# Shigangli/Ok-Topk

Measured on NVIDIA H100. Metric: train_samples_per_sec_vgg16_oktopk_density0.001, higher is better.
Workload: dtype fp32

## Files before the change

### oktopk_b200/config.py

```python
from __future__ import annotations

import dataclasses
from dataclasses import dataclass, field
from typing import Dict, Optional, Sequence


@dataclass
class OkTopkConfig:
    compressor: str = "oktopk"
    density: float = 0.01
    sparse: bool = True

    bucket_elems: int = 64 * 1024 * 1024

    warmup_iters: int = 0
    local_recompute_interval: int = 32
    global_recompute_interval: int = 32
    repartition_interval: int = 64
    topkaopt_recompute_interval: int = 32

    overselect_guard_num: int = 4
    overselect_guard_den: int = 3
    overselect_guard_factor: float = 1.03
    overselect_guard_loops: int = 5
# ... 8 lines not shown
    global_adapt_inc: float = 1.008
    global_adapt_dec: float = 1.008

    throttle: int = 4
    balanced_allgather: bool = False
    dsa_dense_fallback_frac: float = 1.0 / 3.0

    gaussian_low: float = 3.0 / 4.0
    gaussian_high: float = 5.0 / 4.0
    gaussian_factor: float = 1.02
    gaussian_loops: int = 20
    gaussian_mode: str = "vgg"

    sigma_scale: float = 2.5
    norm_clip: Optional[float] = None
    dynamic_densities: Optional[Sequence[float]] = None

    backend: str = "auto"
    fused: bool = True
    deterministic: bool = False
    slot_factor: float = 0.0
    gather_factor: float = 0.0
    dense_switch_density: float = 0.05
    max_redo: int = 12
    redo_factor: float = 1.5
    land_grads: bool = True
    nvls: str = "auto"
    comm_ctas: int = 0
    pull_mode: str = "tma"
    overlap: bool = True
    early_pack: bool = True
    early_pack_frac: float = 0.85
    early_pack_ctas: int = 32
    gselect_mode: str = "auto"
    peer_timeout_s: float = 60.0

    def k_for(self, numel: int, density: Optional[float] = None) -> int:
        d = self.density if density is None else density
        return int(numel * d)

    def replace(self, **kw) -> "OkTopkConfig":
        return dataclasses.replace(self, **kw)

    def to_dict(self) -> Dict:
        return dataclasses.asdict(self)


@dataclass(frozen=True)
class LossScale:
    init_scale: float = 2.0 ** 16
    growth_factor: float = 2.0
    backoff_factor: float = 0.5
    growth_interval: int = 2000

    def __post_init__(self):
        if not (self.init_scale > 0 and self.growth_factor >= 1 and 0 < self.backoff_factor <= 1
                and self.growth_interval >= 1):
            raise ValueError("LossScale: need init_scale > 0, growth_factor >= 1, 0 < backoff_factor <= 1, "
                             "growth_interval >= 1")

    @staticmethod
    def parse(spec) -> Optional["LossScale"]:
        if spec is None or isinstance(spec, LossScale):
            return spec
        if isinstance(spec, str) and spec.strip().lower() == "dynamic":
            return LossScale()
# ... 62 lines not shown
```

### oktopk_b200/csrc/bindings.cpp

```cpp
#include <pybind11/pybind11.h>
#include <pybind11/stl.h>
#include <cuda.h>
#include <cuda_runtime.h>

#include <unistd.h>

#include <algorithm>
#include <cstring>
#include <stdexcept>
#include <string>
#include <tuple>
#include <vector>

#include "oktopk.cuh"

namespace py = pybind11;
using namespace okt;

static void ck(cudaError_t e, const char* what) {
    if (e != cudaSuccess) throw std::runtime_error(std::string(what) + ": " + cudaGetErrorString(e));
}
template <class T> static T* P_(uint64_t p) { return reinterpret_cast<T*>(p); }
static cudaStream_t S_(uint64_t s) { return reinterpret_cast<cudaStream_t>(s); }

// ... 419 lines not shown
    }
}

static void dense_run(const std::vector<uint64_t>& bufs, const std::vector<uint64_t>& flags, uint64_t epoch, int n,
                      int rank, int grid, uint64_t stream, uint64_t st, double timeout_s, uint64_t mc,
                      uint64_t host_fault, uint64_t skip) {
    DenseParams p;
    std::memset(&p, 0, sizeof(p));
    if (bufs.size() > OKT_MAXP || bufs.size() != flags.size()) throw std::runtime_error("bad peer tables");
    for (size_t i = 0; i < bufs.size(); ++i) { p.bufs[i] = P_<float>(bufs[i]); p.flags[i] = P_<uint64_t>(flags[i]); }
    p.epoch = P_<unsigned long long>(epoch);
    p.n = n; p.P = (int)bufs.size(); p.rank = rank; p.scale = 1.0f / (float)p.P;
    p.fault = st ? &P_<OktState>(st)->fault : nullptr;
    p.timeout_ns = (unsigned long long)(timeout_s * 1e9);
    p.mc = P_<float>(mc);
    p.host_fault = P_<int>(host_fault);
    p.skip = P_<const int>(skip);
    ck(launch_dense_allreduce(p, grid, S_(stream)), "dense allreduce launch");
}

static void kth_abs(uint64_t x, int n, int k, uint64_t st, uint64_t out, int grid, uint64_t stream) {
    ck(launch_kth_abs(P_<float>(x), n, k, P_<OktState>(st), P_<float>(out), grid, S_(stream)), "kth_abs launch");
}

static void fused_sgd(uint64_t p, uint64_t g, uint64_t mom, int n, double momentum, double dampening, double wd,
                      int nesterov, int first, int zero_grad, uint64_t stream, uint64_t scal_ptr, uint64_t fault_ptr,
                      uint64_t skip_ptr) {
    if (scal_ptr == 0) throw std::runtime_error("fused_sgd: scal_ptr must point at the group's device scalars");
    ck(launch_fused_sgd(P_<float>(p), P_<float>(g), P_<float>(mom), n, (float)momentum, (float)dampening, (float)wd,
                        nesterov, first, zero_grad, P_<float>(scal_ptr), P_<int>(fault_ptr), P_<int>(skip_ptr),
                        S_(stream)),
       "fused_sgd");
}
static void fused_bert_adam(uint64_t p, uint64_t g, uint64_t m, uint64_t v, int n, double b1, double b2, double eps,
                            double wd, int zero_grad, uint64_t stream, uint64_t scal_ptr, uint64_t fault_ptr,
                            uint64_t skip_ptr) {
    if (scal_ptr == 0) throw std::runtime_error("fused_bert_adam: scal_ptr must point at the group's device scalars");
    ck(launch_fused_bert_adam(P_<float>(p), P_<float>(g), P_<float>(m), P_<float>(v), n, (float)b1, (float)b2,
                              (float)eps, (float)wd, zero_grad, P_<float>(scal_ptr), P_<int>(fault_ptr), P_<int>(skip_ptr),
                              S_(stream)),
       "fused_bert_adam");
}
static void fused_adam(uint64_t p, uint64_t g, uint64_t m, uint64_t v, int n, double beta1, double beta2, double eps,
                       double wd, int decoupled, int zero_grad, uint64_t stream, uint64_t scal_ptr, uint64_t fault_ptr,
                       uint64_t skip_ptr) {
    if (scal_ptr == 0) throw std::runtime_error("fused_adam: scal_ptr must point at the group's device scalars");
    ck(launch_fused_adam(P_<float>(p), P_<float>(g), P_<float>(m), P_<float>(v), n, beta1, beta2, (float)eps, (float)wd,
                         decoupled, zero_grad, P_<float>(scal_ptr), P_<int>(fault_ptr), P_<int>(skip_ptr), S_(stream)),
       "fused_adam");
}
static Dtype dtype_arg(int dtype, const char* what) {
    if (dtype < 0 || dtype > 2) throw std::runtime_error(std::string(what) + ": dtype must be 0 (fp32), 1 (bf16) or 2 (fp16)");
    return static_cast<Dtype>(dtype);
}
static void bn_forward(uint64_t x, uint64_t y, uint64_t arg, uint64_t partial, uint64_t gamma, uint64_t beta, uint64_t cbias,
                       uint64_t save_mean, uint64_t save_invstd, uint64_t rmean, uint64_t rvar, uint64_t nbt, double momentum,
                       double eps, int relu, int M, int C, int W, int slot, int max_ctas, uint64_t stream, int dtype,
                       uint64_t res) {
    if (C % 4 != 0) throw std::runtime_error("bn_forward: channel count must be a multiple of 4");
    if (slot < 0) throw std::runtime_error("bn_forward: negative slot");
    if (res != 0 && (W != 0 || !relu)) throw std::runtime_error("bn_forward: a residual needs relu = 1 and no pool");
    ck(launch_bn_forward(P_<const void>(x), P_<void>(y), P_<unsigned char>(arg), P_<float>(partial), P_<const float>(gamma),
                         P_<const float>(beta), P_<const float>(cbias), P_<float>(save_mean), P_<float>(save_invstd),
                         P_<float>(rmean), P_<float>(rvar), P_<long long>(nbt), (float)momentum, (float)eps, relu, M, C, W, slot,
                         max_ctas, dtype_arg(dtype, "bn_forward"), S_(stream), P_<const void>(res)), "bn_forward");
}
// ... 221 lines not shown
    m.def("max_coop_grid", &okt_max_coop_grid);
    m.def("oktopk_run", &oktopk_run);
    m.def("gather_run", &gather_run);
    m.def("dense_run", &dense_run, py::arg("bufs"), py::arg("flags"), py::arg("epoch"), py::arg("n"), py::arg("rank"),
          py::arg("grid"), py::arg("stream"), py::arg("st") = 0, py::arg("timeout_s") = 0.0, py::arg("mc") = 0,
          py::arg("host_fault") = 0, py::arg("skip") = 0);
    m.def("gtopk_run", &gtopk_run);
    m.def("land_grads", &land_grads);
    m.def("read_trace", &read_trace);
    m.def("host_flag_alloc", &host_flag_alloc);
    m.def("host_flag_free", &host_flag_free);
    m.def("host_flag_read", &host_flag_read);
    m.def("host_flag_clear", &host_flag_clear);
    m.def("fault_ptr", [](uint64_t st) { return (uint64_t)&P_<OktState>(st)->fault; });
    m.def("gather_max_coop_grid", &gather_max_coop_grid);
    m.def("gtopk_max_coop_grid", &gtopk_max_coop_grid);
    m.def("vmm_probe", &vmm_probe);
    m.def("vmm_create", &vmm_create);
    m.def("vmm_import", &vmm_import);
    m.def("vmm_map", &vmm_map);
    m.def("vmm_unmap", &vmm_unmap);
    m.def("vmm_release", &vmm_release);
    m.def("mc_create", &mc_create);
    m.def("mc_add_device", &mc_add_device);
    m.def("mc_bind", &mc_bind);
    m.def("close_fd", [](int fd) { if (fd >= 0) ::close(fd); });
    m.def("clear_fault", [](uint64_t st, uint64_t stream) {
        ck(cudaMemsetAsync(&P_<OktState>(st)->fault, 0, sizeof(int), S_(stream)), "clear_fault");
    });
    m.def("kth_abs", &kth_abs);
    m.def("fused_sgd", &fused_sgd, py::arg("p"), py::arg("g"), py::arg("mom"), py::arg("n"), py::arg("momentum"),
          py::arg("dampening"), py::arg("wd"), py::arg("nesterov"), py::arg("first"), py::arg("zero_grad"),
          py::arg("stream"), py::arg("scal_ptr"), py::arg("fault_ptr") = 0, py::arg("skip_ptr") = 0);
    m.def("fused_bert_adam", &fused_bert_adam, py::arg("p"), py::arg("g"), py::arg("m"), py::arg("v"), py::arg("n"),
          py::arg("b1"), py::arg("b2"), py::arg("eps"), py::arg("wd"), py::arg("zero_grad"), py::arg("stream"),
          py::arg("scal_ptr"), py::arg("fault_ptr") = 0, py::arg("skip_ptr") = 0);
    m.def("fused_adam", &fused_adam, py::arg("p"), py::arg("g"), py::arg("m"), py::arg("v"), py::arg("n"),
          py::arg("beta1"), py::arg("beta2"), py::arg("eps"), py::arg("wd"), py::arg("decoupled"), py::arg("zero_grad"),
          py::arg("stream"), py::arg("scal_ptr"), py::arg("fault_ptr") = 0, py::arg("skip_ptr") = 0);
    m.def("momentum_correct", &momentum_correct);
    m.def("unscale_check", &unscale_check);
    m.def("scale_update", [](uint64_t ls, double growth, double backoff, int interval, uint64_t stream) {
        ck(launch_scale_update(P_<LossScaleDev>(ls), growth, backoff, interval, S_(stream)), "scale_update");
    });
    m.def("adam_scalars", [](uint64_t ls, uint64_t hyper, uint64_t scal, int groups, uint64_t stream) {
        ck(launch_adam_scalars(P_<const LossScaleDev>(ls), P_<const double>(hyper), P_<float>(scal), groups, S_(stream)),
           "adam_scalars");
    });
    m.def("carry_residual", [](uint64_t g, uint64_t res, int n, uint64_t skip, uint64_t stream) {
        ck(launch_carry_residual(P_<float>(g), P_<float>(res), n, P_<const int>(skip), S_(stream)), "carry_residual");
    });
    m.attr("LOSS_SCALE_BYTES") = sizeof(LossScaleDev);
    m.attr("SCALE_SYNC_BYTES") = sizeof(ScaleSync);
    m.attr("VERDICT_OFFSET") = offsetof(ScaleSync, verdict);
    m.def("maxpool2_fwd", &maxpool2_fwd);
    m.def("maxpool2_bwd", &maxpool2_bwd);
    m.def("bn_forward", &bn_forward, py::arg("x"), py::arg("y"), py::arg("arg"), py::arg("partial"), py::arg("gamma"),
          py::arg("beta"), py::arg("cbias"), py::arg("save_mean"), py::arg("save_invstd"), py::arg("rmean"), py::arg("rvar"),
          py::arg("nbt"), py::arg("momentum"), py::arg("eps"), py::arg("relu"), py::arg("M"), py::arg("C"), py::arg("W"),
          py::arg("slot"), py::arg("max_ctas"), py::arg("stream"), py::arg("dtype"), py::arg("res") = 0);
    m.def("bn_backward", &bn_backward, py::arg("x"), py::arg("dy"), py::arg("arg"), py::arg("dx"), py::arg("partial"),
          py::arg("gamma"), py::arg("beta"), py::arg("save_mean"), py::arg("save_invstd"), py::arg("dgamma"), py::arg("dbeta"),
          py::arg("relu"), py::arg("M"), py::arg("C"), py::arg("W"), py::arg("slot"), py::arg("max_ctas"), py::arg("stream"),
          py::arg("dtype"), py::arg("res") = 0, py::arg("dres") = 0);
    m.def("bn_tile_rows", &bn_tile_rows);
    m.def("bn_sliced", &bn_sliced, py::arg("M"), py::arg("C"), py::arg("W"));
// ... 47 lines not shown
```

### oktopk_b200/csrc/oktopk.cuh

```cuda
#pragma once
#include <cuda_runtime.h>
#include <stdint.h>
#include <stddef.h>

#ifndef OKT_MAXP
#define OKT_MAXP 16
#endif

namespace okt {

constexpr int kThreads = 512;
constexpr int kWarps = kThreads / 32;
constexpr int kChunk = 1024;
constexpr int kHistBins = 2048;
constexpr int kMaxWarpsTotal = 16384;
constexpr int kGuardMax = 64;
constexpr int kGuardFineMax = 15;
constexpr int kCtasPerSm = 1;
constexpr int kPackTile = 2;
constexpr int kPackStages = 4;
constexpr int kPackSmemBytes = kPackStages * 2 * kPackTile * kThreads * 16;
constexpr int kScanStages = 2 * kPackStages;
constexpr int kStrideGridMax = 132 * 8;

// ... 194 lines not shown
    int ccap;
    int* sel_idx;
    float* sel_val;
    int selcap;
    int* host_fault;
    const int* skip;
};

struct DenseParams {
    float* bufs[OKT_MAXP];
    uint64_t* flags[OKT_MAXP];
    unsigned long long* epoch;
    int n, P, rank;
    float scale;
    int* fault;
    unsigned long long timeout_ns;
    float* mc;
    int* host_fault;
    const int* skip;
};

int okt_max_coop_grid(int device);
cudaError_t launch_oktopk(const OktParams& p, int grid, cudaStream_t stream);
cudaError_t launch_oktopk_segment(const OktParams& p, int max_ctas, cudaStream_t stream);
cudaError_t launch_gather_scheme(const GatherParams& p, int grid, cudaStream_t stream);
cudaError_t launch_gtopk(const TreeParams& p, int grid, cudaStream_t stream);
int gtopk_max_coop_grid(int device);
int gather_max_coop_grid(int device);
cudaError_t launch_dense_allreduce(const DenseParams& p, int grid, cudaStream_t stream);
cudaError_t launch_kth_abs(const float* x, int n, int k, OktState* st, float* out_thr, int grid, cudaStream_t stream);
cudaError_t launch_fused_sgd(float* p, float* g, float* mom, int n, float momentum, float dampening, float weight_decay,
                             int nesterov, int first_step, int zero_grad, const float* scal, const int* fault,
                             const int* skip, cudaStream_t stream);
cudaError_t launch_fused_bert_adam(float* p, float* g, float* m, float* v, int n, float b1, float b2, float eps,
                                   float weight_decay, int zero_grad, const float* scal, const int* fault,
                                   const int* skip, cudaStream_t stream);
cudaError_t launch_fused_adam(float* p, float* g, float* m, float* v, int n, double beta1, double beta2, float eps,
                              float weight_decay, int decoupled, int zero_grad, const float* scal, const int* fault,
                              const int* skip, cudaStream_t stream);

struct LossScaleDev {
    float scale;
    float inv_scale;
    int growth_tracker;
    int found_inf;
    long long skipped;
    long long adam_step;
};
struct ScaleSync {
    int flag;
    unsigned int ticket;
    unsigned int epoch;
    int verdict;
};
constexpr int kScaleThreads = 256;
constexpr int kScalePerCta = 8192;
struct ScaleParams {
    LossScaleDev* ls;
    ScaleSync* sync;
    int* fault;
    int* host_fault;
    char* peers[OKT_MAXP];
    size_t mbox_off;
    int P, rank;
    unsigned long long timeout_ns;
    int nseg;
// ... 76 lines not shown
```

### oktopk_b200/csrc/optim.cu

```cuda
#include "common.cuh"
#include "oktopk.cuh"

namespace okt {

constexpr int kOptThreads = 256;

template <int kScal, int kState, typename Upd>
__device__ __forceinline__ void update_pass(float* __restrict__ p, float* __restrict__ g, float* __restrict__ m,
                                            float* __restrict__ v, int n, bool load, bool store, int zero_grad,
                                            const float* __restrict__ scal, const int* __restrict__ fault,
                                            const int* __restrict__ skip, Upd upd) {
    if (fault != nullptr && *reinterpret_cast<const volatile int*>(fault) != 0) return;
    const int n4 = n >> 2;
    float4* p4 = reinterpret_cast<float4*>(p);
    float4* g4 = reinterpret_cast<float4*>(g);
    float4* m4 = reinterpret_cast<float4*>(m);
    float4* v4 = reinterpret_cast<float4*>(v);
    const float4 zero = make_float4(0.f, 0.f, 0.f, 0.f);
    if (verdict_set(skip)) {
        if (!zero_grad) return;
        for (int i = blockIdx.x * kOptThreads + threadIdx.x; i < n4; i += gridDim.x * kOptThreads) {
            const float4 gw = ld_stream_f4(g4 + i);
            if (gw.x != 0.f || gw.y != 0.f || gw.z != 0.f || gw.w != 0.f) g4[i] = zero;
        }
// ... 6 lines not shown
    for (int j = 0; j < kScal; ++j) s[j] = scal[j];
    for (int i = blockIdx.x * kOptThreads + threadIdx.x; i < n4; i += gridDim.x * kOptThreads) {
        float4 pw = p4[i], gw = ld_stream_f4(g4 + i), mw = zero, vw = zero;
        if (load) {
            mw = m4[i];
            if (kState == 2) vw = v4[i];
        }
        upd(s, pw.x, gw.x, mw.x, vw.x); upd(s, pw.y, gw.y, mw.y, vw.y);
        upd(s, pw.z, gw.z, mw.z, vw.z); upd(s, pw.w, gw.w, mw.w, vw.w);
        p4[i] = pw;
        if (store) {
            m4[i] = mw;
            if (kState == 2) v4[i] = vw;
        }
        if (zero_grad && (gw.x != 0.f || gw.y != 0.f || gw.z != 0.f || gw.w != 0.f)) g4[i] = zero;
    }
    if (blockIdx.x == 0)
        for (int i = n4 * 4 + threadIdx.x; i < n; i += kOptThreads) {
            float pw = p[i], gw = g[i], mw = 0.f, vw = 0.f;
            if (load) {
                mw = m[i];
                if (kState == 2) vw = v[i];
            }
            upd(s, pw, gw, mw, vw);
            p[i] = pw;
            if (store) {
                m[i] = mw;
                if (kState == 2) v[i] = vw;
            }
            if (zero_grad) g[i] = 0.f;
        }
}

__global__ void __launch_bounds__(kOptThreads) fused_sgd_kernel(float* __restrict__ p, float* __restrict__ g,
                                                                 float* __restrict__ mom, int n, float momentum,
                                                                 float dampening, float wd, int nesterov, int first,
                                                                 int zero_grad, const float* __restrict__ scal,
                                                                 const int* __restrict__ fault,
                                                                 const int* __restrict__ skip) {
    const float damp = first ? 0.f : dampening;
    update_pass<1, 1>(p, g, mom, nullptr, n, momentum != 0.f && !first, momentum != 0.f, zero_grad, scal, fault, skip,
                      [=](const float* s, float& pw, float gw, float& mw, float&) {
                          float d = __fmaf_rn(wd, pw, gw);
                          if (momentum != 0.f) {
                              mw = first ? d : __fmaf_rn(1.f - damp, d, __fmul_rn(momentum, mw));
                              d = nesterov ? __fmaf_rn(momentum, mw, d) : mw;
                          }
                          pw = __fmaf_rn(-s[0], d, pw);
                      });
}

__global__ void __launch_bounds__(kOptThreads) fused_bert_adam_kernel(float* __restrict__ p, float* __restrict__ g,
                                                                       float* __restrict__ m, float* __restrict__ v,
                                                                       int n, float b1, float b2, float eps, float wd,
                                                                       int zero_grad, const float* __restrict__ scal,
                                                                       const int* __restrict__ fault,
                                                                       const int* __restrict__ skip) {
    update_pass<1, 2>(p, g, m, v, n, true, true, zero_grad, scal, fault, skip,
                      [=](const float* s, float& pw, float gw, float& mw, float& vw) {
                          mw = b1 * mw + (1.f - b1) * gw;
                          vw = b2 * vw + (1.f - b2) * gw * gw;
                          float u = mw / (sqrtf(vw) + eps);
                          if (wd > 0.f) u += wd * pw;
                          pw -= s[0] * u;
                      });
}

__global__ void __launch_bounds__(kOptThreads) fused_adam_kernel(float* __restrict__ p, float* __restrict__ g,
                                                                  float* __restrict__ m, float* __restrict__ v, int n,
                                                                  float w, float b2, float omb2, float eps, float wd,
                                                                  int decoupled, int zero_grad,
                                                                  const float* __restrict__ scal,
                                                                  const int* __restrict__ fault,
                                                                  const int* __restrict__ skip) {
    const bool small_w = fabsf(w) < 0.5f;
    const float lw = small_w ? w : 1.f - w;
    update_pass<3, 2>(p, g, m, v, n, true, true, zero_grad, scal, fault, skip,
                      [=](const float* s, float& pw, float gw, float& mw, float& vw) {
                          const float decay = s[0], step_size = s[1], bc2_sqrt = s[2];
                          if (decoupled) pw = pw * decay;
                          else if (wd != 0.f) gw = gw + wd * pw;
                          mw = small_w ? mw + lw * (gw - mw) : gw - (gw - mw) * lw;
// ... 18 lines not shown
    for (int i = blockIdx.x * kOptThreads + threadIdx.x; i < n; i += gridDim.x * kOptThreads) {
        double v = (double)x[i];
        acc += v * v;
    }
    acc = warp_sum_d(acc);
    __shared__ double s[kOptThreads / 32];
    if ((threadIdx.x & 31) == 0) s[threadIdx.x >> 5] = acc;
    __syncthreads();
    if (threadIdx.x < 32) {
        double v = (threadIdx.x < kOptThreads / 32) ? s[threadIdx.x] : 0.0;
        v = warp_sum_d(v);
        if (threadIdx.x == 0) atomicAdd(out, (float)v);
    }
}

__global__ void __launch_bounds__(kOptThreads) clip_scale_kernel(float* __restrict__ x, int n, const float* norm_sq,
                                                                  float max_norm) {
    const float nrm = sqrtf(*norm_sq);
    if (!(nrm > max_norm) || nrm == 0.f) return;
    const float s = max_norm / nrm;
    for (int i = blockIdx.x * kOptThreads + threadIdx.x; i < n; i += gridDim.x * kOptThreads) x[i] *= s;
}

static inline int opt_grid(int n) {
    int g = (n / 4 + kOptThreads - 1) / kOptThreads;
    if (g < 1) g = 1;
    if (g > kStrideGridMax) g = kStrideGridMax;
    return g;
}

cudaError_t launch_fused_sgd(float* p, float* g, float* mom, int n, float momentum, float dampening, float weight_decay,
                             int nesterov, int first_step, int zero_grad, const float* scal, const int* fault,
                             const int* skip, cudaStream_t stream) {
    fused_sgd_kernel<<<opt_grid(n), kOptThreads, 0, stream>>>(p, g, mom, n, momentum, dampening, weight_decay, nesterov,
                                                             first_step, zero_grad, scal, fault, skip);
    return cudaGetLastError();
}

cudaError_t launch_fused_bert_adam(float* p, float* g, float* m, float* v, int n, float b1, float b2, float eps,
                                   float weight_decay, int zero_grad, const float* scal, const int* fault,
                                   const int* skip, cudaStream_t stream) {
    fused_bert_adam_kernel<<<opt_grid(n), kOptThreads, 0, stream>>>(p, g, m, v, n, b1, b2, eps, weight_decay, zero_grad,
                                                                   scal, fault, skip);
    return cudaGetLastError();
}

cudaError_t launch_fused_adam(float* p, float* g, float* m, float* v, int n, double beta1, double beta2, float eps,
                              float weight_decay, int decoupled, int zero_grad, const float* scal, const int* fault,
                              const int* skip, cudaStream_t stream) {
    fused_adam_kernel<<<opt_grid(n), kOptThreads, 0, stream>>>(p, g, m, v, n, (float)(1.0 - beta1), (float)beta2,
                                                              (float)(1.0 - beta2), eps, weight_decay, decoupled,
                                                              zero_grad, scal, fault, skip);
    return cudaGetLastError();
}

constexpr int kLandThreads = 256;
constexpr int kLandPerCta = 8192;

__global__ void __launch_bounds__(kLandThreads) land_kernel(const LandParams lp, float* __restrict__ bucket) {
    int lo = 0, hi = lp.count - 1;
    while (lo < hi) {
        const int mid = (lo + hi + 1) >> 1;
        if ((int)blockIdx.x >= lp.blk_begin[mid]) lo = mid; else hi = mid - 1;
    }
    const int t = lo;
    const int part = blockIdx.x - lp.blk_begin[t];
    const float* __restrict__ src = lp.src[t];
    float* __restrict__ dst = bucket + lp.dst_off[t];
// ... 43 lines not shown
```

### oktopk_b200/ops/ext.py

```python
from __future__ import annotations

import importlib
import os
from typing import Optional

import torch

_C = None
_ERR: Optional[BaseException] = None

LAUNCH_COUNT = {"total": 0}
_LAUNCHERS = {"oktopk_run": 1, "gather_run": 1, "gtopk_run": 1, "dense_run": 1, "kth_abs": 1, "fused_sgd": 1,
              "fused_bert_adam": 1, "fused_adam": 1, "momentum_correct": 1, "clip_by_norm": 2, "land_grads": 1, "bn_forward": 1, "bn_backward": 1,
              "maxpool2_fwd": 1, "maxpool2_bwd": 1, "unscale_check": 1, "ln_forward": 1, "ln_backward": 2,
              "xent_forward": 2, "xent_backward": 1, "lstm_forward": 1, "lstm_backward": 1, "mlm_select": 1,
              "mlm_gather": 1, "mlm_scatter": 1, "attn_forward": 1, "attn_backward": 2, "lstm_seq_forward": 1,
              "lstm_seq_backward": 1}


class _CountingModule:

    def __init__(self, mod):
        self._mod = mod
        for name, per_call in _LAUNCHERS.items():
            setattr(self, name, self._wrap(getattr(mod, name), name, per_call))

    def _wrap(self, fn, name, per_call):
        def call(*a, **kw):
            n = per_call
            if name == "oktopk_run" and isinstance(a[9], dict) and a[9].get("split_phases"):
                n = 7
            if name == "land_grads":
                n = max(1, (len(a[0]) + 95) // 96)
            LAUNCH_COUNT["total"] += n
            LAUNCH_COUNT[name] = LAUNCH_COUNT.get(name, 0) + n
            return fn(*a, **kw)
        return call

    def __getattr__(self, name):
        return getattr(self._mod, name)


def load(build_if_missing: bool = True):
    global _C, _ERR
    if _C is not None:
        return _C
# ... 47 lines not shown
```

### oktopk_b200/optimizer.py

```python
from __future__ import annotations

import math
import warnings
from typing import Dict, Iterable, List, Optional

import torch

from .compression import NoneCompressor, compressors, resolve_compressor
from .config import LossScale, OkTopkConfig
from .ops import ext
from .parallel.allreducer import AllReducer
from .parallel.buckets import Bucket, attach, build_buckets
from .parallel.early_pack import PackPlanner
from .parallel.world import World, world as _world


class _ScaleState:

    def __init__(self, ls: LossScale, device: torch.device):
        self.cfg = ls
        self.buf = torch.zeros(32, dtype=torch.uint8, device=device)
        self.f32 = self.buf[0:8].view(torch.float32)
        self.i32 = self.buf[8:16].view(torch.int32)
        self.i64 = self.buf[16:32].view(torch.int64)
        self.native = device.type == "cuda" and ext.available()
        self.reset()

    @property
    def ptr(self) -> int:
        return self.buf.data_ptr()

    @property
    def found_ptr(self) -> int:
        return self.buf.data_ptr() + 12

    def reset(self, scale: Optional[float] = None, growth_tracker: int = 0, skipped: int = 0, adam_step: int = 0) -> None:
        from .parallel.oracle import inv_scale_of
        scale = self.cfg.init_scale if scale is None else scale
        vals = torch.zeros(32, dtype=torch.uint8)
        vals[0:8].view(torch.float32).copy_(torch.tensor([scale, inv_scale_of(scale)], dtype=torch.float32))
        vals[8:16].view(torch.int32).copy_(torch.tensor([growth_tracker, 0], dtype=torch.int32))
        vals[16:32].view(torch.int64).copy_(torch.tensor([skipped, adam_step], dtype=torch.int64))
        self.buf.copy_(vals)

    def scale(self) -> torch.Tensor:
        return self.f32[0]

# ... 63 lines not shown
        self._use_streams = False
        self._land = False
        for b in self._buckets:
            dev = b.params[0].device
            grad = allreducer.register_bucket(b.name, b.numel, dev)
            attach(b, grad, flatten_params)
            if dev.type == "cuda" and self._cfg.land_grads and ext.available():
                self._land = True
            b.pending = len(b.params)
            b.dirty = False
            if dev.type == "cuda":
                self._use_streams = self._cfg.overlap
                b.event = torch.cuda.Event()
            for p in b.params:
                self._bucket_of[p] = b
                self._hook_handles.append(p.register_post_accumulate_grad_hook(self._make_hook(p)))
        if self._update is _AdamUpdate:
            if not (ext.available() and all(b.flat_param is not None and b.grad.is_cuda for b in self._buckets)):
                self._update = None
        self._direct = (self._land and self._update is not None and allreducer.compressor.name == "oktopk"
                        and all(b.flat_param is not None for b in self._buckets))
        self._packs = {}
        self._pos_in_bucket = {p: i for b in self._buckets for i, p in enumerate(b.params)}
        if self._direct and self._use_streams:
            for b in self._buckets:
                if len(b.params) <= ext.require().SRC_SEG_MAX:
                    self._packs[b.index] = PackPlanner(b.offsets, b.numel,
                                                       math.ceil(self._cfg.early_pack_frac * b.numel),
                                                       ext.require().PACK_RANGE_MAX)
            for b in self._buckets:
                b.packing = None
        if self._use_streams:
            self._comm_stream = torch.cuda.Stream(priority=-1)
        allreducer.add_resync_hook(self._resync_replicas)
        if loss_scale is not None:
            allreducer.enable_loss_scaling()
            self._ls = _ScaleState(loss_scale, self._buckets[0].params[0].device if self._buckets else torch.device("cpu"))
        self._lr_dev = self._hyper_dev = None
        self._lr_pin, self._lr_ev, self._lr_ring, self._lr_last = [], [], 0, None
        dev0 = self._buckets[0].params[0].device if self._buckets else torch.device("cpu")
        if dev0.type == "cuda" and ext.available() and self._update is not None:
            groups = max(len(self.param_groups), 1)
            self._lr_dev = torch.zeros(groups * self._update.n_scalars, dtype=torch.float32, device=dev0)
            stage = self._lr_dev
            if self._ls is not None and self._update is _AdamUpdate:
                stage = self._hyper_dev = torch.zeros(groups * 4, dtype=torch.float64, device=dev0)
            self._lr_pin = [torch.zeros_like(stage, device="cpu").pin_memory() for _ in range(8)]
            self._lr_ev = [None] * len(self._lr_pin)

    def _resync_replicas(self) -> None:
        w = self._allreducer.world
        if w.size == 1:
            return
        for b in self._buckets:
            if b.flat_param is not None:
                w.broadcast(b.flat_param, 0)
            else:
                for p in b.params:
                    w.broadcast(p.data, 0)
            for t in self._flat_state.get(b.index, {}).values():
                if torch.is_tensor(t):
                    w.broadcast(t, 0)

    @property
    def _okt_adam(self) -> bool:
        return self._update is _AdamUpdate
# ... 30 lines not shown
            b = self._bucket_of[p]
            b.dirty = True
            if self.local:
                return
            b.pending -= 1
            if b.pending == 0:
                self._launch_ready()
            elif b.index in self._packs:
                self._pack_early(b, p)
        return hook

    def _pack_early(self, b: Bucket, p) -> None:
        if b.packing is None:
            b.packing = (self._direct and not self.momentum_correction and self._ls is None
                         and self._allreducer.reads_sources(b.name) and self._allreducer.packs_early(b.name))
        if not b.packing:
            return
        planner = self._packs[b.index]
        ranges = planner.ready(self._pos_in_bucket[p])
        if ranges is None:
            return
        ptrs, offs, lens = [], [], []
        for q, o, v in sorted(zip(b.params, b.offsets, b.grad_views), key=lambda t: t[1]):
            g = q.grad
            if not any(lo <= o < hi for lo, hi in ranges) or g is None or g.numel() == 0:
                continue
            if (g.data_ptr() == v.data_ptr() or g.dtype != torch.float32 or not g.is_cuda or g.stride() != v.stride()
                    or g.data_ptr() % 16):
                raise RuntimeError("early pack: the gradient of %s cannot be read in place; set "
                                   "OkTopkConfig.early_pack=False" % self._parameter_names.get(q, "?"))
            ptrs.append(g.data_ptr())
            offs.append(o)
            lens.append(g.numel())
        ev = torch.cuda.Event()
        ev.record(torch.cuda.current_stream())
        self._comm_stream.wait_event(ev)
        with torch.cuda.stream(self._comm_stream):
            self._allreducer.pack_segment(b.name, ranges, (ptrs, offs, lens), stream=self._comm_stream)

    def _launch_ready(self) -> None:
        while self._next_launch < len(self._buckets) and self._buckets[self._next_launch].pending <= 0:
            self._launch(self._buckets[self._next_launch])
            self._next_launch += 1

    def _land_bucket(self, b: Bucket) -> None:
        srcs, offs, numels = [], [], []
        for p, o, v in zip(b.params, b.offsets, b.grad_views):
            g = p.grad
            if g is None:
                srcs.append(0)
                offs.append(o)
                numels.append(p.numel())
            elif g.data_ptr() == v.data_ptr():
                continue
            elif g.dtype == torch.float32 and g.is_cuda and g.stride() == v.stride():
                srcs.append(g.data_ptr())
                offs.append(o)
                numels.append(g.numel())
            else:
                v.copy_(g)
            p.grad = v
        if srcs:
            ext.require().land_grads(srcs, offs, numels, b.grad.data_ptr(), torch.cuda.current_stream().cuda_stream)

    def _source_table(self, b: Bucket):
        ptrs, offs, lens, held = [], [], [], []
        for p, o, v in zip(b.params, b.offsets, b.grad_views):
            g = p.grad
            if g is None or g.numel() == 0:
                continue
            if (g.data_ptr() == v.data_ptr() or g.dtype != torch.float32 or not g.is_cuda or g.stride() != v.stride()
# ... 67 lines not shown
        return loss * self._ls.scale()

    def loss_scale_state(self) -> Optional[Dict]:
        if self._ls is None:
            return None
        st = self._ls.state()
        return {k: st[k] for k in ("scale", "growth_tracker", "skipped_steps")}

    def _scale_state_dict(self) -> Optional[Dict]:
        if self._ls is None:
            return None
        st = self._ls.state()
        st.pop("found_inf")
        return st

    def _load_scale_state(self, sd: Optional[Dict], adam_step: int) -> None:
        if self._ls is None:
            return
        if sd is None:
            self._ls.reset(adam_step=adam_step)
        else:
            self._ls.reset(sd["scale"], sd["growth_tracker"], sd["skipped_steps"], sd.get("adam_step", adam_step))

    def synchronize(self) -> None:
        if self._synced:
            return
        for b in self._buckets:
            b.pending = 0
        self._launch_ready()
        if self._comm_stream is not None:
            cur = torch.cuda.current_stream()
            for b in self._buckets:
                cur.wait_event(b.event)
        for b in self._buckets:
            b.held = None
        self._synced = True

    def _after_step(self) -> None:
        for b in self._buckets:
            b.pending = len(b.params)
            b.launched = False
            if b.index in self._packs:
                self._packs[b.index].reset()
                b.packing = None
        self._next_launch = 0
        self._synced = False
        self._allreducer.poll_faults()

    def _clear_buckets(self) -> None:
        if self._direct:
            with torch.no_grad():
                for b in self._buckets:
                    b.grad.zero_()

    def zero_grad(self, set_to_none: bool = False) -> None:
        if self._land:
            for b in self._buckets:
                for p in b.params:
                    p.grad = None
                b.dirty = False
            return
        for b in self._buckets:
            if b.dirty:
                b.grad.zero_()
                b.dirty = False

    def stop(self) -> None:
        self._allreducer.stop()

    def add_train_epoch(self) -> None:
        self._allreducer.train_epoch += 1

    def get_current_density(self) -> float:
        return self._allreducer.get_current_density()

    def comm_stats(self) -> Dict:
        return self._allreducer.stats()
# ... 23 lines not shown
        else:
            self._maybe_refresh_lr()
            if self._hyper_dev is not None and self._update is _AdamUpdate:
                ext.require().adam_scalars(self._ls.ptr, self._hyper_dev.data_ptr(), self._lr_dev.data_ptr(),
                                           len(self.param_groups), torch.cuda.current_stream().cuda_stream)
            with torch.no_grad():
                for b in self._buckets:
                    self._fused_update(b, host_skip)
            self.counter += 1
        if self._ls is not None:
            self._ls.update()
        self._after_step()
        return loss

    def _device_update(self) -> bool:
        return self._update is not None and self._lr_dev is not None and all(
            b.grad.is_cuda and b.flat_param is not None for b in self._buckets)

    def _flat_buffers(self, b: Bucket) -> Dict[str, torch.Tensor]:
        fs = self._flat_state.setdefault(b.index, {})
        for k in self._update.keys:
            if k not in fs:
                fs[k] = torch.zeros_like(b.grad)
                for p, v in zip(b.params, b.views(fs[k])):
                    self.state[p][k] = v
        return fs

    def _fused_update(self, b: Bucket, host_skip: bool = False) -> None:
        first = self._update.keys[0] not in self._flat_state.get(b.index, {})
        fs = self._flat_buffers(b)
        on_gpu = b.grad.is_cuda and b.flat_param is not None and ext.available()
        zero_grad = 0 if self._land and not self._direct else 1
        skip_ptr = self._ls.found_ptr if self._ls is not None else 0
        for gi, s, e in b.group_slices:
            def launch(fn, *hyper):
                fn(b.flat_param.data_ptr() + 4 * s, b.grad.data_ptr() + 4 * s,
                   *(fs[k].data_ptr() + 4 * s for k in self._update.keys), e - s, *hyper, zero_grad,
                   torch.cuda.current_stream().cuda_stream, self._lr_ptr(gi), self._allreducer.fault_ptr(b.name),
                   skip_ptr)
            if on_gpu or not host_skip:
                self._update.update(self, b, self.param_groups[gi], s, e, fs, first, launch if on_gpu else None)
            if not on_gpu:
                b.grad[s:e].zero_()
        b.dirty = False

    def _adopt_state(self, counter: Optional[int] = None) -> None:
        keys = self._update.keys
        have = {p for b in self._buckets for p in b.params if self.state.get(p, {}).get(keys[0]) is not None}
        if counter is None:
            steps = {float(self.state[p]["step"]) for p in have if "step" in self.state[p]}
            if len(steps) > 1:
                warnings.warn("DistributedOptimizer: the loaded Adam state has unequal step counts per parameter %s; "
                              "using torch's Adam step from now on" % sorted(steps))
                self._update = None
                self._clear_buckets()
                self._direct = False
                for b in self._buckets:
                    for k in keys:
                        self._flat_state.get(b.index, {}).pop(k, None)
                return
            counter = int(steps.pop()) if steps else 0
        self.counter = counter
        loaded = {(p, k): self.state[p][k] for p in have for k in keys}
        with torch.no_grad():
            for b in self._buckets:
                for p in b.params:
                    self.state.get(p, {}).pop("step", None)
                if not any(p in have for p in b.params):
                    for k in keys:
                        self._flat_state.get(b.index, {}).pop(k, None)
                    continue
                fs = self._flat_buffers(b)
                for k in keys:
                    for p, v in zip(b.params, b.views(fs[k])):
                        if p in have:
                            v.copy_(loaded[p, k])
                        else:
                            v.zero_()
                        self.state[p][k] = v


class _SGDUpdate:
    keys = ("momentum_buffer",)
    n_scalars = 1

    @staticmethod
    def scalars(opt, g):
        return (float(g["lr"]),)

    @staticmethod
    def update(opt, b, g, s, e, fs, first, launch):
        lr, m, damp, wd, nest = g["lr"], g.get("momentum", 0.0), g.get("dampening", 0.0), \
            g.get("weight_decay", 0.0), bool(g.get("nesterov", False))
        if opt.momentum_correction:
            m = 0.0
        if launch is not None:
            launch(ext.require().fused_sgd, m, damp, wd, int(nest), int(first))
            return
        gs, ms = b.grad[s:e], fs["momentum_buffer"][s:e]
        if b.flat_param is not None:
            _SGDUpdate.math(b.flat_param[s:e], gs, ms, lr, m, damp, wd, nest, first)
        else:
            for p, o in zip(b.params, b.offsets):
                if s <= o < e:
                    _SGDUpdate.math(p.data.view(-1), gs[o - s:o - s + p.numel()], ms[o - s:o - s + p.numel()],
                                    lr, m, damp, wd, nest, first)

    @staticmethod
    def math(p, g, mom, lr, m, damp, wd, nest, first) -> None:
        d = g.add(p, alpha=wd) if wd != 0 else g.clone()
        if m != 0:
            if first:
                mom.copy_(d)
            else:
                mom.mul_(m).add_(d, alpha=1 - damp)
            d = d.add(mom, alpha=m) if nest else mom
        p.add_(d, alpha=-lr)


class _AdamUpdate:
    keys = ("exp_avg", "exp_avg_sq")
    n_scalars = 3

    @staticmethod
    def scalars(opt, g):
        if opt._hyper_dev is not None:
            return (float(g["lr"]), float(g["weight_decay"]), float(g["betas"][0]), float(g["betas"][1]))
        lr, (b1, b2), t = float(g["lr"]), g["betas"], float(opt.counter + 1)
# ... 235 lines not shown
```

Baseline: 14410.

## Precompute zero-gradient SGD step for early-packed ranges on a side stream

For ranges packed early during backward, a side-stream kernel stashes the params and momentum, then applies the SGD step as if the gradient were zero. It runs limited to a few CTAs so it overlaps with backward and communication. After the allreduce, a tail kernel redoes the update from the stash only where the gradient vector is nonzero, and runs the full update on the remaining dense ranges. This aims to take most of the optimizer's memory traffic off the critical path with very sparse gradients. The cost is two extra stash buffers, added side-stream contention with compute, and extra fault/skip handling that restores the stashed values.

```diff
diff --git a/oktopk_b200/config.py b/oktopk_b200/config.py
--- a/oktopk_b200/config.py
+++ b/oktopk_b200/config.py
@@ -64,6 +64,7 @@
     early_pack: bool = True
     early_pack_frac: float = 0.85
     early_pack_ctas: int = 32
+    sgd_ahead: bool = True
     gselect_mode: str = "auto"
     peer_timeout_s: float = 60.0
 
diff --git a/oktopk_b200/csrc/bindings.cpp b/oktopk_b200/csrc/bindings.cpp
--- a/oktopk_b200/csrc/bindings.cpp
+++ b/oktopk_b200/csrc/bindings.cpp
@@ -475,6 +475,45 @@
                         S_(stream)),
        "fused_sgd");
 }
+static SgdRanges sgd_ranges(const std::vector<std::pair<long long, long long>>& rs, int n, const char* what) {
+    if ((int)rs.size() > kPackRangeMax)
+        throw std::runtime_error(std::string(what) + ": more than " + std::to_string(kPackRangeMax) + " ranges");
+    SgdRanges r;
+    std::memset(&r, 0, sizeof(r));
+    r.nr = (int)rs.size();
+    for (int q = 0; q < r.nr; ++q) {
+        const long long lo = rs[q].first, hi = rs[q].second;
+        if (lo < 0 || hi < lo || lo % 4 || hi % 4 || hi > 4LL * (n / 4))
+            throw std::runtime_error(std::string(what) + ": ranges must lie at multiples of 4 inside the slice's whole "
+                                     "float4 vectors");
+        r.lo[q] = (int)(lo / 4);
+        r.hi[q] = (int)(hi / 4);
+    }
+    return r;
+}
+static void sgd_ahead(uint64_t p, uint64_t mom, uint64_t sp, uint64_t sm, int n,
+                      const std::vector<std::pair<long long, long long>>& ranges, double momentum, double dampening,
+                      double wd, int nesterov, int max_ctas, uint64_t stream, uint64_t scal_ptr) {
+    if (scal_ptr == 0) throw std::runtime_error("sgd_ahead: scal_ptr must point at the group's device scalars");
+    if (momentum != 0.0 && (mom == 0 || sm == 0)) throw std::runtime_error("sgd_ahead: momentum needs mom and sm");
+    const SgdHyper h{(float)momentum, (float)dampening, (float)wd, nesterov, 0};
+    ck(launch_sgd_ahead(P_<float>(p), P_<float>(mom), P_<float>(sp), P_<float>(sm), sgd_ranges(ranges, n, "sgd_ahead"),
+                        h, max_ctas, P_<float>(scal_ptr), S_(stream)),
+       "sgd_ahead");
+}
+static void fused_sgd_tail(uint64_t p, uint64_t g, uint64_t mom, uint64_t sp, uint64_t sm, int n,
+                           const std::vector<std::pair<long long, long long>>& ahead,
+                           const std::vector<std::pair<long long, long long>>& dense, double momentum, double dampening,
+                           double wd, int nesterov, int first, int zero_grad, uint64_t stream, uint64_t scal_ptr,
+                           uint64_t fault_ptr, uint64_t skip_ptr) {
+    if (scal_ptr == 0) throw std::runtime_error("fused_sgd_tail: scal_ptr must point at the group's device scalars");
+    if (momentum != 0.0 && (mom == 0 || sm == 0)) throw std::runtime_error("fused_sgd_tail: momentum needs mom and sm");
+    const SgdHyper h{(float)momentum, (float)dampening, (float)wd, nesterov, first};
+    ck(launch_fused_sgd_tail(P_<float>(p), P_<float>(g), P_<float>(mom), P_<const float>(sp), P_<const float>(sm), n,
+                             sgd_ranges(ahead, n, "fused_sgd_tail"), sgd_ranges(dense, n, "fused_sgd_tail"), h,
+                             zero_grad, P_<float>(scal_ptr), P_<int>(fault_ptr), P_<int>(skip_ptr), S_(stream)),
+       "fused_sgd_tail");
+}
 static void fused_bert_adam(uint64_t p, uint64_t g, uint64_t m, uint64_t v, int n, double b1, double b2, double eps,
                             double wd, int zero_grad, uint64_t stream, uint64_t scal_ptr, uint64_t fault_ptr,
                             uint64_t skip_ptr) {
@@ -762,6 +801,13 @@
     m.def("fused_sgd", &fused_sgd, py::arg("p"), py::arg("g"), py::arg("mom"), py::arg("n"), py::arg("momentum"),
           py::arg("dampening"), py::arg("wd"), py::arg("nesterov"), py::arg("first"), py::arg("zero_grad"),
           py::arg("stream"), py::arg("scal_ptr"), py::arg("fault_ptr") = 0, py::arg("skip_ptr") = 0);
+    m.def("sgd_ahead", &sgd_ahead, py::arg("p"), py::arg("mom"), py::arg("sp"), py::arg("sm"), py::arg("n"),
+          py::arg("ranges"), py::arg("momentum"), py::arg("dampening"), py::arg("wd"), py::arg("nesterov"),
+          py::arg("max_ctas"), py::arg("stream"), py::arg("scal_ptr"));
+    m.def("fused_sgd_tail", &fused_sgd_tail, py::arg("p"), py::arg("g"), py::arg("mom"), py::arg("sp"), py::arg("sm"),
+          py::arg("n"), py::arg("ahead"), py::arg("dense"), py::arg("momentum"), py::arg("dampening"), py::arg("wd"),
+          py::arg("nesterov"), py::arg("first"), py::arg("zero_grad"), py::arg("stream"), py::arg("scal_ptr"),
+          py::arg("fault_ptr") = 0, py::arg("skip_ptr") = 0);
     m.def("fused_bert_adam", &fused_bert_adam, py::arg("p"), py::arg("g"), py::arg("m"), py::arg("v"), py::arg("n"),
           py::arg("b1"), py::arg("b2"), py::arg("eps"), py::arg("wd"), py::arg("zero_grad"), py::arg("stream"),
           py::arg("scal_ptr"), py::arg("fault_ptr") = 0, py::arg("skip_ptr") = 0);
diff --git a/oktopk_b200/csrc/oktopk.cuh b/oktopk_b200/csrc/oktopk.cuh
--- a/oktopk_b200/csrc/oktopk.cuh
+++ b/oktopk_b200/csrc/oktopk.cuh
@@ -250,6 +250,20 @@
 cudaError_t launch_fused_sgd(float* p, float* g, float* mom, int n, float momentum, float dampening, float weight_decay,
                              int nesterov, int first_step, int zero_grad, const float* scal, const int* fault,
                              const int* skip, cudaStream_t stream);
+struct SgdRanges {
+    int nr;
+    int lo[kPackRangeMax];
+    int hi[kPackRangeMax];
+};
+struct SgdHyper {
+    float momentum, dampening, wd;
+    int nesterov, first;
+};
+cudaError_t launch_sgd_ahead(float* p, float* mom, float* sp, float* sm, const SgdRanges& r, const SgdHyper& h,
+                             int max_ctas, const float* scal, cudaStream_t stream);
+cudaError_t launch_fused_sgd_tail(float* p, float* g, float* mom, const float* sp, const float* sm, int n,
+                                  const SgdRanges& ahead, const SgdRanges& dense, const SgdHyper& h, int zero_grad,
+                                  const float* scal, const int* fault, const int* skip, cudaStream_t stream);
 cudaError_t launch_fused_bert_adam(float* p, float* g, float* m, float* v, int n, float b1, float b2, float eps,
                                    float weight_decay, int zero_grad, const float* scal, const int* fault,
                                    const int* skip, cudaStream_t stream);
diff --git a/oktopk_b200/csrc/optim.cu b/oktopk_b200/csrc/optim.cu
--- a/oktopk_b200/csrc/optim.cu
+++ b/oktopk_b200/csrc/optim.cu
@@ -62,22 +62,138 @@
         }
 }
 
+__device__ __forceinline__ void sgd_update(const SgdHyper& h, float lr, float& pw, float gw, float& mw) {
+    const float damp = h.first ? 0.f : h.dampening;
+    float d = __fmaf_rn(h.wd, pw, gw);
+    if (h.momentum != 0.f) {
+        mw = h.first ? d : __fmaf_rn(1.f - damp, d, __fmul_rn(h.momentum, mw));
+        d = h.nesterov ? __fmaf_rn(h.momentum, mw, d) : mw;
+    }
+    pw = __fmaf_rn(-lr, d, pw);
+}
+
+__device__ __forceinline__ void sgd_update4(const SgdHyper& h, float lr, float4& pw, const float4& gw, float4& mw) {
+    sgd_update(h, lr, pw.x, gw.x, mw.x); sgd_update(h, lr, pw.y, gw.y, mw.y);
+    sgd_update(h, lr, pw.z, gw.z, mw.z); sgd_update(h, lr, pw.w, gw.w, mw.w);
+}
+
 __global__ void __launch_bounds__(kOptThreads) fused_sgd_kernel(float* __restrict__ p, float* __restrict__ g,
-                                                                 float* __restrict__ mom, int n, float momentum,
-                                                                 float dampening, float wd, int nesterov, int first,
+                                                                 float* __restrict__ mom, int n, const SgdHyper h,
                                                                  int zero_grad, const float* __restrict__ scal,
                                                                  const int* __restrict__ fault,
                                                                  const int* __restrict__ skip) {
-    const float damp = first ? 0.f : dampening;
-    update_pass<1, 1>(p, g, mom, nullptr, n, momentum != 0.f && !first, momentum != 0.f, zero_grad, scal, fault, skip,
-                      [=](const float* s, float& pw, float gw, float& mw, float&) {
-                          float d = __fmaf_rn(wd, pw, gw);
-                          if (momentum != 0.f) {
-                              mw = first ? d : __fmaf_rn(1.f - damp, d, __fmul_rn(momentum, mw));
-                              d = nesterov ? __fmaf_rn(momentum, mw, d) : mw;
-                          }
-                          pw = __fmaf_rn(-s[0], d, pw);
-                      });
+    update_pass<1, 1>(p, g, mom, nullptr, n, h.momentum != 0.f && !h.first, h.momentum != 0.f, zero_grad, scal, fault,
+                      skip, [=](const float* s, float& pw, float gw, float& mw, float&) { sgd_update(h, s[0], pw, gw, mw); });
+}
+
+constexpr int kAheadUnroll = 4;
+
+__device__ __forceinline__ void st_evict_f4(float4* p, const float4& v) {
+    asm volatile("st.global.cs.v4.f32 [%0], {%1,%2,%3,%4};" ::"l"(p), "f"(v.x), "f"(v.y), "f"(v.z), "f"(v.w) : "memory");
+}
+
+__global__ void __launch_bounds__(kOptThreads) sgd_ahead_kernel(float* __restrict__ p, float* __restrict__ mom,
+                                                                 float* __restrict__ sp, float* __restrict__ sm,
+                                                                 const SgdRanges r, const SgdHyper h,
+                                                                 const float* __restrict__ scal) {
+    const float lr = scal[0];
+    const bool use_m = h.momentum != 0.f;
+    float4* p4 = reinterpret_cast<float4*>(p);
+    float4* m4 = reinterpret_cast<float4*>(mom);
+    float4* sp4 = reinterpret_cast<float4*>(sp);
+    float4* sm4 = reinterpret_cast<float4*>(sm);
+    const float4 zero = make_float4(0.f, 0.f, 0.f, 0.f);
+    const int stride = gridDim.x * kOptThreads;
+    for (int q = 0; q < r.nr; ++q) {
+        const int hi = r.hi[q];
+        for (int i0 = r.lo[q] + blockIdx.x * kOptThreads + threadIdx.x; i0 < hi; i0 += kAheadUnroll * stride) {
+            float4 pw[kAheadUnroll], mw[kAheadUnroll];
+#pragma unroll
+            for (int u = 0; u < kAheadUnroll; ++u) {
+                const int i = i0 + u * stride;
+                pw[u] = mw[u] = zero;
+                if (i < hi) {
+                    pw[u] = ld_stream_f4(p4 + i);
+                    if (use_m) mw[u] = ld_stream_f4(m4 + i);
+                }
+            }
+#pragma unroll
+            for (int u = 0; u < kAheadUnroll; ++u) {
+                const int i = i0 + u * stride;
+                if (i >= hi) continue;
+                st_evict_f4(sp4 + i, pw[u]);
+                if (use_m) st_evict_f4(sm4 + i, mw[u]);
+                sgd_update4(h, lr, pw[u], zero, mw[u]);
+                st_evict_f4(p4 + i, pw[u]);
+                if (use_m) st_evict_f4(m4 + i, mw[u]);
+            }
+        }
+    }
+}
+
+__device__ __forceinline__ bool any_bits(const float4& v) {
+    return (__float_as_uint(v.x) | __float_as_uint(v.y) | __float_as_uint(v.z) | __float_as_uint(v.w)) != 0u;
+}
+
+__global__ void __launch_bounds__(kOptThreads) fused_sgd_tail_kernel(float* __restrict__ p, float* __restrict__ g,
+                                                                      float* __restrict__ mom,
+                                                                      const float* __restrict__ sp,
+                                                                      const float* __restrict__ sm, int n,
+                                                                      const SgdRanges ahead, const SgdRanges dense,
+                                                                      const SgdHyper h, int zero_grad,
+                                                                      const float* __restrict__ scal,
+                                                                      const int* __restrict__ fault,
+                                                                      const int* __restrict__ skip) {
+    const bool use_m = h.momentum != 0.f;
+    float4* p4 = reinterpret_cast<float4*>(p);
+    float4* g4 = reinterpret_cast<float4*>(g);
+    float4* m4 = reinterpret_cast<float4*>(mom);
+    const float4* sp4 = reinterpret_cast<const float4*>(sp);
+    const float4* sm4 = reinterpret_cast<const float4*>(sm);
+    const float4 zero = make_float4(0.f, 0.f, 0.f, 0.f);
+    const int first = blockIdx.x * kOptThreads + threadIdx.x, stride = gridDim.x * kOptThreads;
+    const bool faulted = fault != nullptr && *reinterpret_cast<const volatile int*>(fault) != 0;
+    if (faulted || verdict_set(skip)) {
+        for (int q = 0; q < ahead.nr; ++q)
+            for (int i = ahead.lo[q] + first; i < ahead.hi[q]; i += stride) {
+                p4[i] = sp4[i];
+                if (use_m) m4[i] = sm4[i];
+            }
+        if (faulted) return;
+        update_pass<1, 1>(p, g, mom, nullptr, n, false, false, zero_grad, scal, nullptr, skip,
+                          [](const float*, float&, float, float&, float&) {});
+        return;
+    }
+    const float lr = scal[0];
+    for (int q = 0; q < ahead.nr; ++q)
+        for (int i = ahead.lo[q] + first; i < ahead.hi[q]; i += stride) {
+            const float4 gw = ld_stream_f4(g4 + i);
+            if (!any_bits(gw)) continue;
+            float4 pw = sp4[i], mw = zero;
+            if (use_m) mw = sm4[i];
+            sgd_update4(h, lr, pw, gw, mw);
+            p4[i] = pw;
+            if (use_m) m4[i] = mw;
+            if (zero_grad && (gw.x != 0.f || gw.y != 0.f || gw.z != 0.f || gw.w != 0.f)) g4[i] = zero;
+        }
+    for (int q = 0; q < dense.nr; ++q)
+        for (int i = dense.lo[q] + first; i < dense.hi[q]; i += stride) {
+            float4 pw = p4[i], gw = ld_stream_f4(g4 + i), mw = zero;
+            if (use_m && !h.first) mw = m4[i];
+            sgd_update4(h, lr, pw, gw, mw);
+            p4[i] = pw;
+            if (use_m) m4[i] = mw;
+            if (zero_grad && (gw.x != 0.f || gw.y != 0.f || gw.z != 0.f || gw.w != 0.f)) g4[i] = zero;
+        }
+    if (blockIdx.x == 0)
+        for (int i = (n >> 2) * 4 + threadIdx.x; i < n; i += kOptThreads) {
+            float pw = p[i], gw = g[i], mw = 0.f;
+            if (use_m && !h.first) mw = mom[i];
+            sgd_update(h, lr, pw, gw, mw);
+            p[i] = pw;
+            if (use_m) mom[i] = mw;
+            if (zero_grad) g[i] = 0.f;
+        }
 }
 
 __global__ void __launch_bounds__(kOptThreads) fused_bert_adam_kernel(float* __restrict__ p, float* __restrict__ g,
@@ -162,8 +278,28 @@
 cudaError_t launch_fused_sgd(float* p, float* g, float* mom, int n, float momentum, float dampening, float weight_decay,
                              int nesterov, int first_step, int zero_grad, const float* scal, const int* fault,
                              const int* skip, cudaStream_t stream) {
-    fused_sgd_kernel<<<opt_grid(n), kOptThreads, 0, stream>>>(p, g, mom, n, momentum, dampening, weight_decay, nesterov,
-                                                             first_step, zero_grad, scal, fault, skip);
+    const SgdHyper h{momentum, dampening, weight_decay, nesterov, first_step};
+    fused_sgd_kernel<<<opt_grid(n), kOptThreads, 0, stream>>>(p, g, mom, n, h, zero_grad, scal, fault, skip);
+    return cudaGetLastError();
+}
+
+cudaError_t launch_sgd_ahead(float* p, float* mom, float* sp, float* sm, const SgdRanges& r, const SgdHyper& h,
+                             int max_ctas, const float* scal, cudaStream_t stream) {
+    if (h.first) return cudaErrorInvalidValue;
+    long long vecs = 0;
+    for (int q = 0; q < r.nr; ++q) vecs += r.hi[q] - r.lo[q];
+    if (vecs <= 0) return cudaSuccess;
+    long long grid = (vecs + kOptThreads * kAheadUnroll - 1) / (kOptThreads * kAheadUnroll);
+    grid = std::min<long long>(grid, std::max(max_ctas, 1));
+    sgd_ahead_kernel<<<(int)grid, kOptThreads, 0, stream>>>(p, mom, sp, sm, r, h, scal);
+    return cudaGetLastError();
+}
+
+cudaError_t launch_fused_sgd_tail(float* p, float* g, float* mom, const float* sp, const float* sm, int n,
+                                  const SgdRanges& ahead, const SgdRanges& dense, const SgdHyper& h, int zero_grad,
+                                  const float* scal, const int* fault, const int* skip, cudaStream_t stream) {
+    fused_sgd_tail_kernel<<<opt_grid(n), kOptThreads, 0, stream>>>(p, g, mom, sp, sm, n, ahead, dense, h, zero_grad,
+                                                                  scal, fault, skip);
     return cudaGetLastError();
 }
 
diff --git a/oktopk_b200/ops/ext.py b/oktopk_b200/ops/ext.py
--- a/oktopk_b200/ops/ext.py
+++ b/oktopk_b200/ops/ext.py
@@ -11,7 +11,7 @@
 
 LAUNCH_COUNT = {"total": 0}
 _LAUNCHERS = {"oktopk_run": 1, "gather_run": 1, "gtopk_run": 1, "dense_run": 1, "kth_abs": 1, "fused_sgd": 1,
-              "fused_bert_adam": 1, "fused_adam": 1, "momentum_correct": 1, "clip_by_norm": 2, "land_grads": 1, "bn_forward": 1, "bn_backward": 1,
+              "sgd_ahead": 1, "fused_sgd_tail": 1, "fused_bert_adam": 1, "fused_adam": 1, "momentum_correct": 1, "clip_by_norm": 2, "land_grads": 1, "bn_forward": 1, "bn_backward": 1,
               "maxpool2_fwd": 1, "maxpool2_bwd": 1, "unscale_check": 1, "ln_forward": 1, "ln_backward": 2,
               "xent_forward": 2, "xent_backward": 1, "lstm_forward": 1, "lstm_backward": 1, "mlm_select": 1,
               "mlm_gather": 1, "mlm_scatter": 1, "attn_forward": 1, "attn_backward": 2, "lstm_seq_forward": 1,
diff --git a/oktopk_b200/optimizer.py b/oktopk_b200/optimizer.py
--- a/oktopk_b200/optimizer.py
+++ b/oktopk_b200/optimizer.py
@@ -1,6 +1,7 @@
 from __future__ import annotations
 
 import math
+import os
 import warnings
 from typing import Dict, Iterable, List, Optional
 
@@ -13,6 +14,9 @@
 from .parallel.buckets import Bucket, attach, build_buckets
 from .parallel.early_pack import PackPlanner
 from .parallel.world import World, world as _world
+
+
+SGD_AHEAD_CTAS = 24
 
 
 class _ScaleState:
@@ -142,6 +146,18 @@
                 b.packing = None
         if self._use_streams:
             self._comm_stream = torch.cuda.Stream(priority=-1)
+        self._ahead_stash: Dict[int, tuple] = {}
+        self._ahead_stream = None
+        self._ahead_ctas = SGD_AHEAD_CTAS
+        if (self._packs and self._update is _SGDUpdate and self._cfg.sgd_ahead
+                and os.environ.get("OKTOPK_SGD_AHEAD", "1") != "0"):
+            self._ahead_stream = torch.cuda.Stream()
+            for b in self._buckets:
+                if b.index in self._packs:
+                    mom = any(self.param_groups[gi].get("momentum", 0.0) != 0 for gi, _, _ in b.group_slices)
+                    self._ahead_stash[b.index] = (torch.empty_like(b.grad), torch.empty_like(b.grad) if mom else None)
+        for b in self._buckets:
+            b.ahead = None
         allreducer.add_resync_hook(self._resync_replicas)
         if loss_scale is not None:
             allreducer.enable_loss_scaling()
@@ -238,11 +254,33 @@
             ptrs.append(g.data_ptr())
             offs.append(o)
             lens.append(g.numel())
+        if b.ahead is None:
+            b.ahead = b.index in self._ahead_stash and self._update.keys[0] in self._flat_state.get(b.index, {})
+            if b.ahead:
+                self._maybe_refresh_lr()
         ev = torch.cuda.Event()
         ev.record(torch.cuda.current_stream())
         self._comm_stream.wait_event(ev)
         with torch.cuda.stream(self._comm_stream):
             self._allreducer.pack_segment(b.name, ranges, (ptrs, offs, lens), stream=self._comm_stream)
+        if b.ahead:
+            self._sgd_ahead(b, ranges, ev)
+
+    def _sgd_ahead(self, b: Bucket, ranges, ev) -> None:
+        s_ = self._ahead_stream
+        if s_ is not self._comm_stream:
+            s_.wait_event(ev)
+        sp, sm = self._ahead_stash[b.index]
+        fs = self._flat_state[b.index]
+        C = ext.require()
+        for gi, s, e in b.group_slices:
+            rs = _clip_ranges(ranges, s, e)
+            if not rs:
+                continue
+            m, damp, wd, nest = _SGDUpdate.hyper(self, self.param_groups[gi])
+            C.sgd_ahead(b.flat_param.data_ptr() + 4 * s, fs["momentum_buffer"].data_ptr() + 4 * s, sp.data_ptr() + 4 * s,
+                        sm.data_ptr() + 4 * s if sm is not None else 0, e - s, rs, m, damp, wd, int(nest),
+                        int(self._ahead_ctas), s_.cuda_stream, self._lr_ptr(gi))
 
     def _launch_ready(self) -> None:
         while self._next_launch < len(self._buckets) and self._buckets[self._next_launch].pending <= 0:
@@ -376,6 +414,8 @@
             cur = torch.cuda.current_stream()
             for b in self._buckets:
                 cur.wait_event(b.event)
+            if any(b.ahead for b in self._buckets):
+                cur.wait_stream(self._ahead_stream)
         for b in self._buckets:
             b.held = None
         self._synced = True
@@ -387,6 +427,7 @@
             if b.index in self._packs:
                 self._packs[b.index].reset()
                 b.packing = None
+            b.ahead = None
         self._next_launch = 0
         self._synced = False
         self._allreducer.poll_faults()
@@ -476,6 +517,10 @@
         on_gpu = b.grad.is_cuda and b.flat_param is not None and ext.available()
         zero_grad = 0 if self._land and not self._direct else 1
         skip_ptr = self._ls.found_ptr if self._ls is not None else 0
+        if b.ahead and on_gpu:
+            self._sgd_tail(b, fs, zero_grad, skip_ptr)
+            b.dirty = False
+            return
         for gi, s, e in b.group_slices:
             def launch(fn, *hyper):
                 fn(b.flat_param.data_ptr() + 4 * s, b.grad.data_ptr() + 4 * s,
@@ -487,6 +532,21 @@
             if not on_gpu:
                 b.grad[s:e].zero_()
         b.dirty = False
+
+    def _sgd_tail(self, b: Bucket, fs: Dict[str, torch.Tensor], zero_grad: int, skip_ptr: int) -> None:
+        planner = self._packs[b.index]
+        ahead = [r for seg in planner.segments for r in seg]
+        rest = planner.rest()
+        sp, sm = self._ahead_stash[b.index]
+        C = ext.require()
+        for gi, s, e in b.group_slices:
+            m, damp, wd, nest = _SGDUpdate.hyper(self, self.param_groups[gi])
+            C.fused_sgd_tail(b.flat_param.data_ptr() + 4 * s, b.grad.data_ptr() + 4 * s,
+                             fs["momentum_buffer"].data_ptr() + 4 * s, sp.data_ptr() + 4 * s,
+                             sm.data_ptr() + 4 * s if sm is not None else 0, e - s, _clip_ranges(ahead, s, e),
+                             _clip_ranges(rest, s, e), m, damp, wd, int(nest), 0, zero_grad,
+                             torch.cuda.current_stream().cuda_stream, self._lr_ptr(gi),
+                             self._allreducer.fault_ptr(b.name), skip_ptr)
 
     def _adopt_state(self, counter: Optional[int] = None) -> None:
         keys = self._update.keys
@@ -524,6 +584,16 @@
                         self.state[p][k] = v
 
 
+def _clip_ranges(ranges, s: int, e: int):
+    top = 4 * ((e - s) // 4)
+    out = []
+    for lo, hi in ranges:
+        lo, hi = max(lo - s, 0), min(hi - s, top)
+        if lo < hi:
+            out.append((lo, hi))
+    return out
+
+
 class _SGDUpdate:
     keys = ("momentum_buffer",)
     n_scalars = 1
@@ -533,11 +603,14 @@
         return (float(g["lr"]),)
 
     @staticmethod
+    def hyper(opt, g):
+        m = 0.0 if opt.momentum_correction else g.get("momentum", 0.0)
+        return m, g.get("dampening", 0.0), g.get("weight_decay", 0.0), bool(g.get("nesterov", False))
+
+    @staticmethod
     def update(opt, b, g, s, e, fs, first, launch):
-        lr, m, damp, wd, nest = g["lr"], g.get("momentum", 0.0), g.get("dampening", 0.0), \
-            g.get("weight_decay", 0.0), bool(g.get("nesterov", False))
-        if opt.momentum_correction:
-            m = 0.0
+        lr = g["lr"]
+        m, damp, wd, nest = _SGDUpdate.hyper(opt, g)
         if launch is not None:
             launch(ext.require().fused_sgd, m, damp, wd, int(nest), int(first))
             return
```

Result: faster. 15000 (median of 6 runs) (+4.1%).
